# andres-fr/realtime-pose-estimation

Hardware: AMD Instinct MI355X
Metric: images/sec at 640x640 (HRNet-w48 fwd+decode) (higher is better)
Workload: dtype f16 (fp32 accumulate, fp32 BatchNorm; fp32 NCHW in/out); 1 GPU; configs[2]: batch=32 per GPU, 640x640, half-wrapper teacher forward + decode of 17 keypoint channels, weights W0 (seeded random); batch_per_gpu=32, people_per_batch_rank0=960

## Files before the change

realtime-pose-estimation_amd/csrc/conv_mfma.hip:

```cpp
#include <vector>

#include "rtpe_common.h"

namespace rtpe {

typedef _Float16 half8 __attribute__((ext_vector_type(8)));
typedef _Float16 half4 __attribute__((ext_vector_type(4)));
typedef float float4v __attribute__((ext_vector_type(4)));

constexpr int kTapTableBytes = 2048;

__device__ __forceinline__ float round16(float v) { return (float)(_Float16)v; }

template <typename T> struct Prec;
template <> struct Prec<_Float16> {
  static constexpr int EPS = 8;
  static __device__ __forceinline__ float rnd(float v) { return (float)(_Float16)v; }
};
template <> struct Prec<float> {
  static constexpr int EPS = 4;
  static __device__ __forceinline__ float rnd(float v) { return v; }
};

template <typename T>
// ... 532 lines not shown
#define RTPE_CONV_MIXED_VARIANTS(V)                                                                     \
  V(3, 8, 4) V(3, 4, 4) V(3, 2, 4) V(3, 5, 4) V(3, 5, 5) V(4, 4, 4) V(4, 2, 4) V(4, 5, 4) V(4, 5, 5) V(6, 2, 4)   \
  V(2, 8, 4) V(2, 4, 4) V(2, 2, 4) V(2, 5, 4) V(2, 5, 5) V(1, 8, 4) V(1, 4, 4) V(1, 2, 4) V(1, 5, 4) V(1, 5, 5)

static bool conv_has_variant(int mt, int nt, int waves) {
#define RTPE_V(MTv, NTv, Wv) if (mt == MTv && nt == NTv && waves == Wv) return true;
  RTPE_CONV_VARIANTS(RTPE_V)
#undef RTPE_V
  return false;
}

struct TileCand { int waves, nt, th, tw; };
static const TileCand kCands[] = {
    {4, 8, 16, 32}, {4, 8, 32, 16}, {4, 4, 16, 16}, {4, 4, 8, 32}, {4, 4, 32, 8},
    {4, 2, 8, 16},  {4, 2, 16, 8},  {5, 5, 20, 20}, {5, 5, 10, 40}, {5, 5, 40, 10},
    {4, 5, 16, 20}, {4, 5, 20, 16}, {4, 5, 8, 40},  {4, 5, 40, 8},
    {4, 1, 8, 8},
    {2, 2, 8, 8}, {1, 4, 8, 8},
};

static size_t tile_lds(const ConvPlan& p, int th, int tw, int waves, int nt, int mrun = 0) {
  const int hh = (th - 1) * p.in_mul + (p.tapw - 1) * p.dil + 1;
  const size_t in_tile = (size_t)hh * conv_row_pitch(p, tw, 0);
  const size_t out_tile = (size_t)waves * nt * 16 * ((mrun ? (mrun > 0 ? mrun : -mrun) : p.mt) * 16 * p.esize + 16);
  return (size_t)kTapTableBytes + (in_tile > out_tile ? in_tile : out_tile);
}

static bool stream_tile(const ConvPlan& p, const TileCand& c, int N, int H_pos, int W_pos, ConvTile* out,
                        bool allow_resident = true) {
  if (!conv_stream_supports(p) || c.waves < 4) return false;
  if (p.in_mul == 1 ? (c.nt != 4 && c.nt != 5) : (c.nt != (p.mt == 6 ? 1 : 2) || p.n_cchunks != 1)) return false;
  if (p.mt == 6 && p.in_mul != 2) return false;
  const int hh = (c.th - 1) * p.in_mul + 3, hw = (c.tw - 1) * p.in_mul + 3;
  if (hw * 6 > 256) return false;
  const size_t in_tile = (size_t)hh * conv_row_pitch(p, c.tw, 2);
  const size_t out_tile = (size_t)c.waves * c.nt * 16 * (p.mt * 32 + 16);
  size_t buf = in_tile > out_tile ? in_tile : out_tile;
  buf = (buf + 255) / 256 * 256;
  int nw = 3, nb = 3;
  if (allow_resident && p.n_cchunks <= 2 && conv_stream_lds(p, (int)buf, 2, 2 * p.n_cchunks) <= 160 * 1024)
    nw = 2 * p.n_cchunks;
  if (conv_stream_lds(p, (int)buf, nb, nw) > 160 * 1024) nb = 2;
  if (conv_stream_lds(p, (int)buf, nb, nw) > 160 * 1024) return false;
  const long tiles = (long)((H_pos + c.th - 1) / c.th) * ((W_pos + c.tw - 1) / c.tw) * N;
  const long units = tiles * p.n_cb;
  static const int g_env = env_int("RTPE_PERSIST_G", 32);
  long G = g_env;
  const long need = (units + 7) / 8;
  if (G > need) G = need;
  G = (G + p.n_cb - 1) / p.n_cb * p.n_cb;
  memset(out, 0, sizeof(*out));
  out->nt = c.nt; out->waves = c.waves; out->th = c.th; out->tw = c.tw;
  out->kind = 2; out->grid = (int)(8 * G); out->buf_bytes = (int)buf; out->n_bufs = nb;
  out->n_wslots = nw;
  out->lds_bytes = conv_stream_lds(p, (int)buf, nb, nw);
  return true;
}

static ConvTile make_stream_tile(const ConvPlan& p, int N, int H_pos, int W_pos) {
  static const int force_nt = RTPE_DIAG_ENV_INT("RTPE_CONV_NT", 0);
  static const int force_waves = RTPE_DIAG_ENV_INT("RTPE_CONV_WAVES", 0);
  static const int force_th = RTPE_DIAG_ENV_INT("RTPE_CONV_TH", 0);
  double best_score = 1e30;
  ConvTile best;
  memset(&best, 0, sizeof(best));
  for (const TileCand& c : kCands) {
    ConvTile t;
    if ((force_nt && c.nt != force_nt) || (force_waves && c.waves != force_waves) || (force_th && c.th != force_th)) continue;
    if (!stream_tile(p, c, N, H_pos, W_pos, &t)) continue;
    const double waste = (double)((H_pos + c.th - 1) / c.th * c.th) * ((W_pos + c.tw - 1) / c.tw * c.tw) /
                         ((double)H_pos * W_pos);
// ... 39 lines not shown
  static const int stream = getenv("RTPE_CONV_STREAM") ? atoi(getenv("RTPE_CONV_STREAM")) : 1;
  if (allow_stream && (stream & 1) && conv_stream_supports(p)) {
    ConvTile t = make_stream_tile(p, N, H_pos, W_pos);
    if (t.nt) return t;
  }
  static const long lds_cap = getenv("RTPE_CONV_LDS_CAP") ? atol(getenv("RTPE_CONV_LDS_CAP")) : 80 * 1024;
  static const int force_nt = RTPE_DIAG_ENV_INT("RTPE_CONV_NT", 0);
  static const int force_waves = RTPE_DIAG_ENV_INT("RTPE_CONV_WAVES", 0);
  double best_score = 1e30;
  ConvTile best;
  memset(&best, 0, sizeof(best));
  for (const TileCand& c : kCands) {
    if (p.mt == 4 && c.nt == 8) continue;
    if (p.mt == 6 && c.nt > 2) continue;
    if (c.nt == 1 || c.waves < 4) continue;
    if (force_nt && c.nt != force_nt) continue;
    if (force_waves && c.waves != force_waves) continue;
    const size_t lds = tile_lds(p, c.th, c.tw, c.waves, c.nt);
    if (lds > 160 * 1024 || ((long)lds > lds_cap && !(c.nt == 2))) continue;
    const long tiles = (long)((H_pos + c.th - 1) / c.th) * ((W_pos + c.tw - 1) / c.tw);
    const double waste = (double)tiles * c.th * c.tw / ((double)H_pos * W_pos);
    const long wgs = tiles * N * p.n_cb;
    double score = waste;
    if (wgs < 512) score *= 1.0 + 0.25 * (512.0 - wgs) / 512.0;
    score *= 1.0 + 0.4 / c.nt;
    const double halo = (double)((c.th - 1) * p.in_mul + (p.tapw - 1) * p.dil + 1) *
                        ((c.tw - 1) * p.in_mul + (p.tapw - 1) * p.dil + 1) / ((double)c.th * c.tw * p.in_mul * p.in_mul);
    score *= 1.0 + 0.1 * (halo - 1.0);
    if (score < best_score) {
      best_score = score;
// ... 128 lines not shown
      ConvTile st;
      if (stream_tile(p, c, N, H_pos, W_pos, &st)) out->push_back(st);
      if (p.n_cchunks == 2 && st.nt && st.n_wslots != 3 && stream_tile(p, c, N, H_pos, W_pos, &st, false) &&
          st.n_bufs == 3)
        out->push_back(st);
    }
  }
  {
    ConvTile dt;
    if (direct_tile(p, &dt)) out->push_back(dt);
    if (conv64_tile(p, N, H_pos, W_pos, &dt)) out->push_back(dt);
  }
}

int conv_launch(const ConvPlan& p, const ConvTile& t, const ConvArgs& a, hipStream_t s) {
  RTPE_REQUIRE(t.th * t.tw * (t.kind == 0 && t.mrun < 0 ? 2 : 1) == 16 * t.nt * t.waves,
               "conv tile %dx%d != 16*%d*%d", t.th, t.tw, t.nt, t.waves);
  RTPE_REQUIRE(t.lds_bytes <= 160 * 1024, "conv tile needs %zu B of LDS", t.lds_bytes);
  RTPE_REQUIRE(t.kind != 0 || t.lds_bytes >= tile_lds(p, t.th, t.tw, t.waves, t.nt, t.mrun),
               "conv tile (%zu B of LDS) was made for another plan (needs %zu B)", t.lds_bytes,
               tile_lds(p, t.th, t.tw, t.waves, t.nt, t.mrun));
  RTPE_REQUIRE(a.kc * 4 * sizeof(int) <= (size_t)kTapTableBytes, "k chunk table overflow (kc=%d)", a.kc);
  const int eps = 16 / p.esize;
  RTPE_REQUIRE(a.in_ld % eps == 0 && (a.y == nullptr || (a.out_ld % eps == 0 && a.cout_store % eps == 0 &&
                                                         ((uintptr_t)a.y & 15) == 0)),
               "conv: NHWC views must be 16-byte aligned with channel counts that are multiples of %d "
               "(in_ld=%d out_ld=%d cout_store=%d y=%p)", eps, a.in_ld, a.out_ld, a.cout_store, (void*)a.y);
  RTPE_REQUIRE(a.res == nullptr || (a.res_ld % eps == 0 && ((uintptr_t)a.res & 15) == 0), "conv: residual view alignment");
  RTPE_REQUIRE(((uintptr_t)a.x & 15) == 0, "conv: input view must be 16-byte aligned");
  if (t.kind == 2) return conv_stream_launch(p, t, a, s);
  if (t.kind == 4) return conv_direct_launch(p, a, s);
// ... 31 lines not shown
```

realtime-pose-estimation_amd/csrc/conv_stream.hip:

```cpp
#include "conv_stream_dev.h"

namespace rtpe {


constexpr int kResReg0 = 224;
#define RTPE_RES_LOAD(K, R0, R1, R2, R3)                                                             \
  if (it == K)                                                                                       \
    asm volatile("global_load_dwordx4 v[" #R0 ":" #R3 "], %0, %1" ::"v"(off), "s"(rb)               \
                 : "memory", "v" #R0, "v" #R1, "v" #R2, "v" #R3);
#define RTPE_RES_ADD(K, R0, R1, R2, R3)                                                              \
  if (it == K)                                                                                       \
    asm volatile("v_pk_add_f16 %0, %0, v" #R0 "\n\tv_pk_add_f16 %1, %1, v" #R1 "\n\tv_pk_add_f16 %2, %2, v" #R2 \
                 "\n\tv_pk_add_f16 %3, %3, v" #R3                                                   \
                 : "+v"(w[0]), "+v"(w[1]), "+v"(w[2]), "+v"(w[3]));
#define RTPE_RES_ALL(X)                                                                              \
  X(0, 224, 225, 226, 227) X(1, 228, 229, 230, 231) X(2, 232, 233, 234, 235) X(3, 236, 237, 238, 239) \
  X(4, 240, 241, 242, 243) X(5, 244, 245, 246, 247) X(6, 248, 249, 250, 251) X(7, 252, 253, 254, 255)

template <int MT, int NT, int WAVES>
__global__ void __launch_bounds__((WAVES + kLoaders) * 64) __attribute__((amdgpu_num_vgpr(kResReg0)))
conv_stream_kernel(const ConvArgs a) {
  extern __shared__ __attribute__((aligned(16))) char smem[];
  constexpr int WSLOT = MT * kKH * 1024;
  char* const wring = smem;
  const int NWS = a.n_wslots;
  char* const tiles = smem + NWS * WSLOT;
  const int tid = threadIdx.x;
  const int lane = tid & 63;
  const int wv = __builtin_amdgcn_readfirstlane(tid >> 6);

  Units um;
  um.init(a.N * a.tiles_x * a.tiles_y, a.n_cb);
  const uint32_t tiles_xy = (uint32_t)(a.tiles_x * a.tiles_y);
  const int ncc = a.n_cchunks;
  const int sh = __builtin_ctz((unsigned)ncc);
  const int S = um.count << sh;
// ... 150 lines not shown
#endif
    return;
  }

  const int r = lane & 15;
  const int g = lane >> 4;
  int toff[kKC];
#pragma unroll
  for (int k = 0; k < kKC; ++k) {
    int kk = k * 32 + g * 8;
    if (kk >= 9 * kCC) kk -= 9 * kCC;
    const int tap = kk / kCC, c = kk - tap * kCC;
    const int ty = tap / 3, tx = tap - ty * 3;
    toff[k] = ty * a.rowb + tx * kPStride + c * 2;
  }
  int pixbase[NT];
#pragma unroll
  for (int nt = 0; nt < NT; ++nt) {
    const uint32_t p = (wv * NT + nt) * 16 + r;
    const uint32_t oy = fdiv(p, a.div_tw);
    const uint32_t ox = p - oy * a.tw;
    pixbase[nt] = (int)(oy * a.in_mul * a.rowb + ox * a.in_mul * kPStride);
  }
  constexpr int ROWB = MT * 32 + 16;
  constexpr int CH = MT * 2;
  constexpr int NIT = (NT * 16 * CH + 63) / 64;
  int eoff[NIT], epos[NIT];
#pragma unroll
  for (int it = 0; it < NIT; ++it) {
    const int c = it * 64 + lane;
    const int pw = c / CH, slot = c - pw * CH;
    const uint32_t p = wv * NT * 16 + pw;
    const uint32_t oyt = fdiv(p, a.div_tw);
    const uint32_t oxt = p - oyt * a.tw;
    eoff[it] = c < NT * 16 * CH ? pw * ROWB + slot * 16 : 0;
    epos[it] = (int)((oyt << 16) | ((oxt * a.o_mul) << 8) | (slot * 16));
  }
  const uint32_t row_pix = (uint32_t)(a.W_full * a.o_mul) & 0xffffffu;
  auto piece_off = [&](int e, uint32_t ld2) __attribute__((always_inline)) {
    const uint32_t pix = __umul24((uint32_t)e >> 16, row_pix) + (((uint32_t)e >> 8) & 255u);
    return __umul24(pix, ld2) + ((uint32_t)e & 255u);
  };

  float4v acc[MT][NT];
  int bsel = 0;
  int wsel = 0;
  const int n_units = um.count;

  float4v al[MT], be[MT];
  int cb0;
  {
    int tile0;
    um.get(0, &tile0, &cb0);
#pragma unroll
    for (int m = 0; m < MT; ++m) {
      const int c4 = (cb0 * MT + m) * 16 + g * 4;
      al[m] = *reinterpret_cast<const float4v*>(a.alpha + c4);
      be[m] = *reinterpret_cast<const float4v*>(a.beta + c4);
    }
  }
#pragma unroll
  for (int m = 0; m < MT; ++m)
    asm volatile("" ::"v"(al[m]), "v"(be[m]));
  const int cblk = cb0 * MT * 16;
#pragma unroll
  for (int it = 0; it < NIT; ++it) {
    const int c = it * 64 + lane;
    const int slot = c % CH;
    if (c >= NT * 16 * CH || cblk + slot * 8 >= a.cout_store) epos[it] |= 0x7fff0000;
  }
  const bool use_res = a.res != nullptr && !(a.ablate & 2);
#ifdef RTPE_CONV_STAMPS
  unsigned long long st[16] = {0};
  const unsigned long long k_begin = __builtin_readcyclecounter();
#endif

  auto half_stage = [&](const char* wslot, const char* tilebuf, auto hsel) {
    constexpr int H = decltype(hsel)::value;
    const char* wl = wslot + lane * 16;
    half8 af[2][MT], bf[2][NT];
#pragma unroll
    for (int m = 0; m < MT; ++m) af[0][m] = *reinterpret_cast<const half8*>(wl + m * 1024);
#pragma unroll
    for (int nt = 0; nt < NT; ++nt) bf[0][nt] = *reinterpret_cast<const half8*>(tilebuf + pixbase[nt] + toff[H * kKH]);
#pragma unroll
    for (int kk = 0; kk < kKH; ++kk) {
      const int cur = kk & 1, nxt = cur ^ 1;
      if (kk + 1 < kKH) {
#pragma unroll
        for (int m = 0; m < MT; ++m)
          af[nxt][m] = *reinterpret_cast<const half8*>(wl + ((kk + 1) * MT + m) * 1024);
#pragma unroll
        for (int nt = 0; nt < NT; ++nt)
          bf[nxt][nt] = *reinterpret_cast<const half8*>(tilebuf + pixbase[nt] + toff[H * kKH + kk + 1]);
      }
#pragma unroll
      for (int m = 0; m < MT; ++m)
#pragma unroll
        for (int nt = 0; nt < NT; ++nt)
          acc[m][nt] = __builtin_amdgcn_mfma_f32_16x16x32_f16(af[cur][m], bf[cur][nt], acc[m][nt], 0, 0, 0);
      if (kk + 1 < kKH) {
#pragma unroll
        for (int i = 0; i < (MT + NT + 3) / 4; ++i) {
          __builtin_amdgcn_sched_group_barrier(0x008, 1, 0);
          __builtin_amdgcn_sched_group_barrier(0x002, 4, 0);
          __builtin_amdgcn_sched_group_barrier(0x100, 4, 0);
        }
      }
      __builtin_amdgcn_sched_barrier(0);
    }
  };

  struct UnitPos { uint32_t n; int py0, px0; };
  auto unit_pos = [&](int u) {
    int tile, cb;
    um.get(u, &tile, &cb);
    uint32_t t = (uint32_t)tile;
    UnitPos q;
    q.n = fdiv(t, a.div_tiles_xy);
    t -= q.n * tiles_xy;
    const uint32_t tyi = fdiv(t, a.div_tiles_x);
    const uint32_t txi = t - tyi * a.tiles_x;
    q.py0 = (int)tyi * a.th;
    q.px0 = (int)txi * a.tw;
    return q;
  };
  static_assert(NIT <= 8, "residual register window");
  auto load_res = [&](int u) {
    const UnitPos q = unit_pos(u);
    const int hy = a.H_pos - q.py0, hx = (a.W_pos - q.px0) * a.o_mul;
    const size_t pix0 = ((size_t)q.n * a.H_full + q.py0 * a.o_mul + a.oy_add) * a.W_full + q.px0 * a.o_mul + a.ox_add;
    const _Float16* rb = a.res + pix0 * a.res_ld + (size_t)cb0 * a.res_cs;
    const uint32_t ld2 = (uint32_t)a.res_ld * 2u;
#pragma unroll
    for (int it = 0; it < NIT; ++it) {
      int e = epos[it];
      asm volatile("" : "+v"(e));
      const bool ok = (e >> 16) < hy && ((e >> 8) & 255) < hx;
      const uint32_t off = ok ? piece_off(e, ld2) : 0u;
      RTPE_RES_ALL(RTPE_RES_LOAD)
    }
  };

  auto run_unit = [&](int u) {
#ifdef RTPE_CONV_STAMPS
    unsigned long long m0, m1, m2, m3, m4;
#endif
    const UnitPos q = unit_pos(u);
#pragma unroll
    for (int m = 0; m < MT; ++m)
#pragma unroll
      for (int nt = 0; nt < NT; ++nt) acc[m][nt] = float4v{0.f, 0.f, 0.f, 0.f};
    char* tilebuf = nullptr;
    for (int cci = 0; cci < ncc; ++cci) {
      tilebuf = tiles + bsel * a.buf_bytes;
      const int w0 = resident ? 2 * cci : wsel;
      const int w1 = resident ? 2 * cci + 1 : (wsel == 2 ? 0 : wsel + 1);
      SSTAMP(m0);
      RTPE_SBARRIER();
      SSTAMP(m1);
      if (!(a.ablate & 1)) half_stage(wring + w0 * WSLOT, tilebuf, std::integral_constant<int, 0>());
      SSTAMP(m2);
      if (!resident) RTPE_SBARRIER();
      SSTAMP(m3);
      if (!(a.ablate & 1)) half_stage(wring + w1 * WSLOT, tilebuf, std::integral_constant<int, 1>());
      SSTAMP(m4);
#ifdef RTPE_CONV_STAMPS
      st[0] += m1 - m0; st[1] += m2 - m1; st[2] += m3 - m2; st[3] += m4 - m3; st[5] += 1;
#endif
      if (cci + 1 < ncc) {
        bsel = bsel + 1 == NB ? 0 : bsel + 1;
        wsel = wsel == 0 ? 2 : wsel - 1;
      }
    }
    int lane_e = lane;
    asm volatile("" : "+v"(lane_e));
    const int re = lane_e & 15, ge = lane_e >> 4;
    asm volatile("s_waitcnt lgkmcnt(0)" ::: "memory");
    SSTAMP(m0);
    RTPE_SBARRIER();
    SSTAMP(m1);
    char* obuf = tilebuf + wv * (NT * 16 * ROWB);
    auto bn_to_lds = [&](auto rc, auto nchw) {
      constexpr bool RC = decltype(rc)::value, NCHW = decltype(nchw)::value;
#pragma unroll
      for (int nt = 0; nt < NT; ++nt) {
#pragma unroll
        for (int m = 0; m < MT; ++m) {
          const float4v v = acc[m][nt];
          half4 o;
          if (RC) {
            o = bn_round(v, al[m], be[m]);
          } else {
            float2v lo{v[0], v[1]}, hi{v[2], v[3]};
            lo = __builtin_elementwise_fma(lo, float2v{al[m][0], al[m][1]}, float2v{be[m][0], be[m][1]});
            hi = __builtin_elementwise_fma(hi, float2v{al[m][2], al[m][3]}, float2v{be[m][2], be[m][3]});
            const half2v olo = __builtin_convertvector(lo, half2v), ohi = __builtin_convertvector(hi, half2v);
            o = half4{olo[0], olo[1], ohi[0], ohi[1]};
          }
          *reinterpret_cast<half4*>(obuf + (nt * 16 + re) * ROWB + m * 32 + ge * 8) = o;
          if (NCHW) {
            const uint32_t p = (wv * NT + nt) * 16 + re;
            const uint32_t oyt = fdiv(p, a.div_tw);
            const uint32_t oxt = p - oyt * a.tw;
            const int py = q.py0 + (int)oyt, px = q.px0 + (int)oxt;
            if (py < a.H_pos && px < a.W_pos) {
              const int oy = py * a.o_mul + a.oy_add, ox = px * a.o_mul + a.ox_add;
              const int c4 = (cb0 * MT + m) * 16 + ge * 4;
#pragma unroll
              for (int jx = 0; jx < 4; ++jx) {
                const int c = c4 + jx;
                if (c < a.nchw_channels) {
                  const float xr = (float)o[jx];
                  const float x = a.relu ? (xr > 0.f ? xr : 0.f) : xr;
                  const size_t oi = (((size_t)q.n * a.nchw_channels + c) * a.H_full + oy) * a.W_full + ox;
                  if (a.nchw_f32)
                    reinterpret_cast<float*>(a.y_nchw)[oi] = x;
                  else
                    reinterpret_cast<_Float16*>(a.y_nchw)[oi] = (_Float16)x;
                }
              }
            }
          }
        }
      }
    };
    if (a.y_nchw != nullptr) {
      if (a.round_conv) bn_to_lds(std::true_type(), std::true_type()); else bn_to_lds(std::false_type(), std::true_type());
    } else {
      if (a.round_conv) bn_to_lds(std::true_type(), std::false_type()); else bn_to_lds(std::false_type(), std::false_type());
    }
    SSTAMP(m2);
    if (a.y != nullptr && !(a.ablate & 2)) {
      if (use_res) asm volatile("s_waitcnt vmcnt(0)" ::: "memory");
      SSTAMP(m3);
      half8 ov[NIT];
#pragma unroll
      for (int it = 0; it < NIT; ++it) ov[it] = *reinterpret_cast<const half8*>(obuf + eoff[it]);
      const int hy = a.H_pos - q.py0, hx = (a.W_pos - q.px0) * a.o_mul;
      const size_t pix0 = ((size_t)q.n * a.H_full + q.py0 * a.o_mul + a.oy_add) * a.W_full + q.px0 * a.o_mul + a.ox_add;
      char* const yb = reinterpret_cast<char*>(a.y + pix0 * a.out_ld + (size_t)cb0 * a.out_cs);
      const uint32_t ld2 = (uint32_t)a.out_ld * 2u;
#pragma unroll
      for (int it = 0; it < NIT; ++it) {
        if (use_res) {
          int4v w = __builtin_bit_cast(int4v, ov[it]);
          RTPE_RES_ALL(RTPE_RES_ADD)
          ov[it] = __builtin_bit_cast(half8, w);
        }
        if (a.relu) {
          short8 b = __builtin_bit_cast(short8, ov[it]);
          b = b & ~(b >> 15);
          ov[it] = __builtin_bit_cast(half8, b);
        }
      }
      if (use_res && u + 1 < n_units) load_res(u + 1);
#pragma unroll
      for (int it = 0; it < NIT; ++it) {
        int e = epos[it];
        asm volatile("" : "+v"(e));
        if ((e >> 16) < hy && ((e >> 8) & 255) < hx) store16_wt(yb + piece_off(e, ld2), ov[it]);
      }
    }
    asm volatile("s_waitcnt lgkmcnt(0)" ::: "memory");
    SSTAMP(m4);
#ifdef RTPE_CONV_STAMPS
    { unsigned long long m5; SSTAMP(m5);
      st[12] += m1 - m0; st[13] += m2 - m1; st[4] += m3 - m2; st[14] += m4 - m3; st[10] += m5 - m4; }
#endif
    bsel = bsel + 1 == NB ? 0 : bsel + 1;
    wsel = wsel == 0 ? 2 : wsel - 1;
  };

  if ((a.ablate >> 8) && ((blockIdx.x >> 3) & 1))
    for (int i = 0; i < (a.ablate >> 8); ++i) __builtin_amdgcn_s_sleep(16);
  if (use_res) load_res(0);
  for (int u = 0; u < n_units; ++u) run_unit(u);
#ifdef RTPE_CONV_STAMPS
  if (a.dbg != nullptr && lane == 0) {
    st[15] = __builtin_readcyclecounter() - k_begin;
    const int slots[] = {0, 1, 2, 3, 4, 5, 10, 12, 13, 14, 15};
    for (int i : slots) atomicAdd(&a.dbg[i], st[i]);
  }
#endif
}

template <int MT, int NT, int WAVES>
static int launch_stream(const ConvTile& t, const ConvArgs& a, hipStream_t s) {
  static unsigned long long attr_mask = 0;
  auto kern = conv_stream_kernel<MT, NT, WAVES>;
  if (first_use_on_device(&attr_mask)) {
    RTPE_HIP_CHECK(hipFuncSetAttribute(reinterpret_cast<const void*>(kern),
                                       hipFuncAttributeMaxDynamicSharedMemorySize, 160 * 1024));
  }
  hipLaunchKernelGGL(kern, dim3((unsigned)t.grid), dim3((WAVES + kLoaders) * 64), t.lds_bytes, s, a);
  RTPE_HIP_CHECK(hipGetLastError());
  return RTPE_OK;
}

size_t conv_stream_lds(const ConvPlan& p, int buf_bytes, int n_bufs, int n_wslots) {
  return (size_t)n_wslots * p.mt * kKH * 1024 + (size_t)n_bufs * buf_bytes;
}

bool conv_stream_supports(const ConvPlan& p) {
  return p.esize == 2 && p.dil == 1 && p.cc == kCC && p.pstride == kPStride && p.tapw == 3 && p.kc == kKC &&
         (p.in_mul == 1 || p.in_mul == 2) && (p.mt <= 3 || (p.mt == 6 && p.in_mul == 2 && p.n_cchunks == 1)) &&
         (p.n_cchunks & (p.n_cchunks - 1)) == 0;
}

int conv_stream_launch(const ConvPlan& p, const ConvTile& t, const ConvArgs& a, hipStream_t s) {
  RTPE_REQUIRE(conv_stream_supports(p), "streaming conv: unsupported plan");
  RTPE_REQUIRE(a.x_bytes > 0 && a.x_bytes < 0x80000000ull, "streaming conv: input view of %zu bytes", (size_t)a.x_bytes);
  RTPE_REQUIRE(a.cin % 8 == 0 && (a.in_ld >= a.cin ? a.in_cs == kCC : a.in_ld == kCC && a.in_cs >= kCC),
               "streaming conv: cin=%d in_ld=%d chunk stride %lld", a.cin, a.in_ld, a.in_cs);
  RTPE_REQUIRE(t.grid >= 8 && t.grid % 8 == 0 && (t.grid / 8) % p.n_cb == 0, "streaming conv: bad grid %d", t.grid);
  RTPE_REQUIRE((t.n_bufs == 2 || t.n_bufs == 3) && t.buf_bytes % 16 == 0 &&
               (t.n_wslots == 3 || t.n_wslots == 2 * p.n_cchunks) &&
               t.lds_bytes >= conv_stream_lds(p, t.buf_bytes, t.n_bufs, t.n_wslots) && t.lds_bytes <= 160 * 1024,
               "streaming conv: LDS layout (%d buffers of %d B, %d weight slots, %zu B)", t.n_bufs, t.buf_bytes,
               t.n_wslots, t.lds_bytes);
  RTPE_REQUIRE(a.halo_w * kSlots <= 256, "streaming conv: halo row of %d pixels", a.halo_w);
  RTPE_REQUIRE(a.rowb >= a.halo_w * kPStride && (size_t)a.halo_h * a.rowb <= (size_t)t.buf_bytes &&
               (size_t)t.waves * t.nt * 16 * (p.mt * 32 + 16) <= (size_t)t.buf_bytes, "streaming conv: tile buffer too small");
#define RTPE_S(MTv, NTv, Wv) \
  if (p.mt == MTv && t.nt == NTv && t.waves == Wv) return launch_stream<MTv, NTv, Wv>(t, a, s);
  RTPE_S(3, 4, 4) RTPE_S(3, 5, 4) RTPE_S(3, 5, 5) RTPE_S(3, 2, 4) RTPE_S(6, 1, 4)
  RTPE_S(2, 4, 4) RTPE_S(2, 5, 4) RTPE_S(2, 5, 5)
  RTPE_S(1, 4, 4) RTPE_S(1, 5, 4) RTPE_S(1, 5, 5)
#undef RTPE_S
  set_error("streaming conv: no kernel variant mt=%d nt=%d waves=%d", p.mt, t.nt, t.waves);
  return RTPE_E_INVALID;
}

}
```

realtime-pose-estimation_amd/csrc/engine.hip:

```cpp
#include <stdarg.h>

#include <chrono>
#include <mutex>
#include <map>
#include <tuple>
#include <vector>

#include "rtpe_common.h"

namespace rtpe {

static thread_local std::string g_err;

void set_error(const char* fmt, ...) {
  char buf[1024];
  va_list ap;
  va_start(ap, fmt);
  vsnprintf(buf, sizeof(buf), fmt, ap);
  va_end(ap);
  g_err = buf;
}

int hip_fail(hipError_t e, const char* what, const char* file, int line) {
  set_error("HIP error %d (%s) at %s:%d: %s", (int)e, hipGetErrorString(e), file, line, what);
// ... 54 lines not shown
  size_t arena_bytes;
  int n_preds, n_refined;
  std::mutex lane_mu;
  hipStream_t lane_stream[4] = {nullptr, nullptr, nullptr, nullptr};
  std::vector<hipEvent_t> op_event;
  std::vector<char> needs_event;
  std::vector<std::vector<int>> wait_ops;
  hipEvent_t fork_event = nullptr;
  bool has_regions = false;
  bool any_size = false;
};

static size_t align_up(size_t v, size_t a) { return (v + a - 1) / a * a; }

namespace rtpe {
static int g_options[kNumOptions] = {-1, -1, -1, -1, -1, -1, -1, -1, -1, -1, -1, -1};
static const char* const kOptionNames[kNumOptions] = {"block_ring", "block_pc", "direct_1x1", "lanes", "tile_dma", "pair_1x1", "fused_stem", "conv64", "head_direct", "deconv48", "conv48s2", "pair_proj"};
static const char* const kOptionEnv[kNumOptions] = {"RTPE_BLOCK_RING", "RTPE_BLOCK_PC", "RTPE_DIRECT_1X1", "RTPE_LANES", "RTPE_TILE_DMA", "RTPE_PAIR_1X1", "RTPE_FUSED_STEM", "RTPE_CONV64", "RTPE_HEAD_DIRECT", "RTPE_DECONV48", "RTPE_CONV48S2", "RTPE_PAIR_PROJ"};
static const int kOptionDefault[kNumOptions] = {0, 1, 1, 1, 1, 1, 1, 1, 1, 1, 1, 1};
int get_option(int key) {
  int v = __atomic_load_n(&g_options[key], __ATOMIC_RELAXED);
  if (v < 0) {
    v = kOptionEnv[key][0] ? env_int(kOptionEnv[key], kOptionDefault[key]) : kOptionDefault[key];
    __atomic_store_n(&g_options[key], v, __ATOMIC_RELAXED);
  }
  return v;
}
}

extern "C" int rtpe_set_option(const char* name, int32_t value) {
  RTPE_REQUIRE(name != nullptr && value >= 0, "set_option: bad argument");
  for (int k = 0; k < kNumOptions; ++k)
    if (kOptionNames[k][0] && strcmp(name, kOptionNames[k]) == 0) {
      __atomic_store_n(&g_options[k], (int)value, __ATOMIC_RELAXED);
// ... 400 lines not shown
    if (!(plane[d.in_t] || plane[d.out_t] || (d.res_t >= 0 && plane[d.res_t]))) continue;
    const rtpe_tensor_desc& ti = h->tensors[d.in_t];
    const ConvTile t = (tuned && (*tuned)[i * 4].nt) ? (*tuned)[i * 4]
                                                      : conv_make_tile(o.plan[0], N, extent(H, ti.ds_log2), extent(W, ti.ds_log2));
    if (t.kind != 2) {
      plane[d.in_t] = plane[d.out_t] = 0;
      if (d.res_t >= 0) plane[d.res_t] = 0;
    }
  }
  return plane;
}

struct RouteOpts {
  int fused_stem = get_option(kOptFusedStem), pair_1x1 = get_option(kOptPair1x1), pair_proj = get_option(kOptPairProj),
      conv64 = get_option(kOptConv64), head_direct = get_option(kOptHeadDirect), deconv48 = get_option(kOptDeconv48),
      conv48s2 = get_option(kOptConv48s2);
};

struct Fwd {
  const rtpe_hrnet* h;
  int N, H, W;
  char* base;
  void *preds, *refined;
  int out_dtype;
  std::vector<size_t> offs;
  size_t ws_need;
  const std::vector<ConvTile>* tuned = nullptr;
  std::vector<char> plane;
  bool rag;
  const int32_t* ext;
  const int32_t* level(int ds) const { return ext + (size_t)ds * 2 * N; }
// ... 86 lines not shown
static ConvArgs conv_op_args(const Fwd& f, size_t i, int k, const ConvTile& t) {
  ConvArgs a = conv_op_args(f, i, k);
  conv_fill_args(f.h->ops[i].geom[k], f.h->ops[i].plan[k], t, &a);
  return a;
}

static bool conv_direct_ok(const ConvArgs& a) {
  return a.x_bytes < 0x80000000ull && a.y != nullptr && a.y_nchw == nullptr && a.o_mul == 1;
}

static void conv_fix_tile(const RouteOpts& opt, const ConvPlan& p, const ConvArgs& a, bool plane_io, ConvTile* t) {
  const bool direct_ok = conv_direct_ok(a);
  if (t->kind == 4 && !direct_ok) *t = conv_make_tile(p, a.N, a.H_pos, a.W_pos, false);
  if (t->kind == 5 && !(direct_ok && a.res == nullptr && !plane_io && opt.conv64 != 0))
    *t = conv_make_tile(p, a.N, a.H_pos, a.W_pos, true, false);
}

static int conv_pick(const RouteOpts& opt, const ConvPlan& p, const ConvTile& t, const ConvArgs& a, bool plane_io) {
  if (opt.head_direct != 0 && conv_head_supports(p, a)) return kRouteHead;
  if (opt.conv48s2 != 0 && !plane_io && conv48s2_supports(p, a)) return kRouteS2;
  return t.kind == 2 ? kRouteStream : t.kind == 4 ? kRouteDirect : t.kind == 5 ? kRouteConv64 : kRouteTile;
}

static bool deconv_merges(const ConvPlan* p, const ConvTile& tile0) {
  static const int merge_deconv = env_int("RTPE_DECONV_MERGE", 1);
  bool merge = merge_deconv && tile0.kind == 0;
  for (int k = 1; k < 4 && merge; ++k)
    merge = p[k].mt == p[0].mt && p[k].cc == p[0].cc && p[k].kc == p[0].kc && p[k].n_cchunks == p[0].n_cchunks &&
            p[k].n_cb == p[0].n_cb && p[k].pstride == p[0].pstride && p[k].tapw == p[0].tapw;
  return merge;
// ... 1099 lines not shown
```

realtime-pose-estimation_amd/csrc/rtpe_common.h:

```cpp
#pragma once
#include <hip/hip_runtime.h>
#include <hip/hip_fp16.h>
#include <stdint.h>
#include <stdio.h>
#include <stdlib.h>
#include <string.h>
#include <string>
#include <vector>

#include "rtpe_hip.h"

namespace rtpe {

void set_error(const char* fmt, ...);
int hip_fail(hipError_t e, const char* what, const char* file, int line);

#define RTPE_HIP_CHECK(expr)                                               \
  do {                                                                     \
    hipError_t _e = (expr);                                                \
    if (_e != hipSuccess) return ::rtpe::hip_fail(_e, #expr, __FILE__, __LINE__); \
  } while (0)

#define RTPE_REQUIRE(cond, ...)                 \
  do {                                          \
// ... 1 lines not shown
      ::rtpe::set_error(__VA_ARGS__);           \
      return RTPE_E_INVALID;                    \
    }                                           \
  } while (0)

inline int env_int(const char* name, int dflt) {
  const char* v = getenv(name);
  return v ? atoi(v) : dflt;
}
#ifdef RTPE_DIAG
#define RTPE_DIAG_ENV_INT(name, dflt) ::rtpe::env_int(name, dflt)
#else
#define RTPE_DIAG_ENV_INT(name, dflt) (dflt)
#endif

enum { kOptBlockRing = 0, kOptBlockPC = 1, kOptDirect1x1 = 2, kOptLanes = 3, kOptTileDma = 4, kOptPair1x1 = 5, kOptFusedStem = 6, kOptConv64 = 7, kOptHeadDirect = 8, kOptDeconv48 = 9, kOptConv48s2 = 10, kOptPairProj = 11, kNumOptions = 12 };
int get_option(int key);

inline bool first_use_on_device(unsigned long long* mask) {
  int dev = 0;
  if (hipGetDevice(&dev) != hipSuccess || dev < 0 || dev > 63) return true;
  const unsigned long long bit = 1ull << dev;
  const unsigned long long old = __atomic_fetch_or(mask, bit, __ATOMIC_RELAXED);
  return !(old & bit);
}

struct DeviceGuard {
  int prev = -1;
  bool switched = false;
  hipError_t err = hipSuccess;
  explicit DeviceGuard(int device) {
// ... 130 lines not shown
  int deconv_class;
  int esize;
  int dil;
};

ConvPlan conv_make_plan(const ConvGeom& g);
ConvTile conv_make_tile(const ConvPlan& p, int N, int H_pos, int W_pos, bool allow_direct = true, bool allow_conv64 = true,
                        bool allow_stream = true);
int conv_row_pitch(const ConvPlan& p, int tw, int kind);
bool conv_deint(const ConvPlan& p, int kind);
void conv_enum_tiles(const ConvPlan& p, int N, int H_pos, int W_pos, std::vector<ConvTile>* out);
void conv_pack_weights(const ConvGeom& g, const ConvPlan& p, const void* w, void* packed);
void conv_fill_args(const ConvGeom& g, const ConvPlan& p, const ConvTile& t, ConvArgs* a);
int conv_launch(const ConvPlan& p, const ConvTile& t, const ConvArgs& a, hipStream_t s);
bool conv_stream_supports(const ConvPlan& p);
size_t conv_stream_lds(const ConvPlan& p, int buf_bytes, int n_bufs, int n_wslots);
int conv_stream_launch(const ConvPlan& p, const ConvTile& t, const ConvArgs& a, hipStream_t s);
bool conv_pair_supports(int cin1, int cout1, int cout2);
int conv_pair_launch(const ConvPlan& p1, const ConvArgs& c1, const ConvPlan& p2, const ConvArgs& c2, hipStream_t s,
                     const ConvPlan* pd = nullptr, const ConvArgs* cd = nullptr);
int conv_direct_mb(const ConvPlan& p);
bool conv64_supports(const ConvPlan& p);
size_t conv64_lds();
int conv64_grid(int N, int H_pos, int W_pos);
int conv64_launch(const ConvPlan& p, const ConvTile& t, const ConvArgs& a, hipStream_t s);
int conv_direct_launch(const ConvPlan& p, const ConvArgs& a, hipStream_t s);
bool conv_head_supports(const ConvPlan& p, const ConvArgs& a);
int conv_head_launch(const ConvPlan& p, const ConvArgs& a, hipStream_t s);
bool deconv48_supports(const ConvPlan& p, const ConvArgs& merged);
int deconv48_launch(const ConvPlan& p, const ConvArgs& merged, hipStream_t s);
// ... 80 lines not shown
```

Measured before the change: 2395 images/sec.

## Add split streaming-conv tile using four waves for 400-pixel 48-channel tiles

Adds a split variant of the streaming 3x3 conv kernel for stride-1, 48-channel cout blocks. Four compute waves each take six 16-pixel column tiles, and the leftover 25th column tile is spread across three waves, one cout subtile each, using a rotated weight order. This replaces the five-wave 20x20-style tiles with four waves and drops a wave per workgroup. The cost is an extra MFMA stream per wave, a late residual and BN load, and extra LDS for the odd slab. The option is on by default and swaps in via a resplit when a five-wave tile was chosen.

```diff
diff --git a/realtime-pose-estimation_amd/csrc/conv_mfma.hip b/realtime-pose-estimation_amd/csrc/conv_mfma.hip
--- a/realtime-pose-estimation_amd/csrc/conv_mfma.hip
+++ b/realtime-pose-estimation_amd/csrc/conv_mfma.hip
@@ -570,6 +570,7 @@
 static const TileCand kCands[] = {
     {4, 8, 16, 32}, {4, 8, 32, 16}, {4, 4, 16, 16}, {4, 4, 8, 32}, {4, 4, 32, 8},
     {4, 2, 8, 16},  {4, 2, 16, 8},  {5, 5, 20, 20}, {5, 5, 10, 40}, {5, 5, 40, 10},
+    {4, kStreamSplitNt, 20, 20}, {4, kStreamSplitNt, 10, 40}, {4, kStreamSplitNt, 40, 10},
     {4, 5, 16, 20}, {4, 5, 20, 16}, {4, 5, 8, 40},  {4, 5, 40, 8},
     {4, 1, 8, 8},
     {2, 2, 8, 8}, {1, 4, 8, 8},
@@ -583,14 +584,18 @@
 }
 
 static bool stream_tile(const ConvPlan& p, const TileCand& c, int N, int H_pos, int W_pos, ConvTile* out,
-                        bool allow_resident = true) {
+                        bool allow_resident = true, int split_mode = -1) {
   if (!conv_stream_supports(p) || c.waves < 4) return false;
-  if (p.in_mul == 1 ? (c.nt != 4 && c.nt != 5) : (c.nt != (p.mt == 6 ? 1 : 2) || p.n_cchunks != 1)) return false;
+  const bool split = c.nt == kStreamSplitNt;
+  if (split && !(p.in_mul == 1 && p.mt == 3)) return false;
+  if (p.in_mul == 1 && p.mt == 3 && (split || c.waves == 5) &&
+      split != ((split_mode < 0 ? get_option(kOptStreamSplit) : split_mode) != 0)) return false;
+  if (p.in_mul == 1 ? (c.nt != 4 && c.nt != 5 && !split) : (c.nt != (p.mt == 6 ? 1 : 2) || p.n_cchunks != 1)) return false;
   if (p.mt == 6 && p.in_mul != 2) return false;
   const int hh = (c.th - 1) * p.in_mul + 3, hw = (c.tw - 1) * p.in_mul + 3;
   if (hw * 6 > 256) return false;
   const size_t in_tile = (size_t)hh * conv_row_pitch(p, c.tw, 2);
-  const size_t out_tile = (size_t)c.waves * c.nt * 16 * (p.mt * 32 + 16);
+  const size_t out_tile = conv_stream_slab(p, c.waves, c.nt);
   size_t buf = in_tile > out_tile ? in_tile : out_tile;
   buf = (buf + 255) / 256 * 256;
   int nw = 3, nb = 3;
@@ -611,6 +616,20 @@
   out->n_wslots = nw;
   out->lds_bytes = conv_stream_lds(p, (int)buf, nb, nw);
   return true;
+}
+
+void conv_stream_resplit(const ConvPlan& p, int N, int H_pos, int W_pos, bool split, ConvTile* t) {
+  if (t->kind != 2 || p.in_mul != 1 || p.mt != 3) return;
+  const bool is = conv_stream_is_split(*t);
+  if (is == split || (!is && t->waves != 5)) return;
+  for (const TileCand& c : kCands) {
+    if (c.th != t->th || c.tw != t->tw || (c.nt == kStreamSplitNt) != split || (!split && c.waves != 5)) continue;
+    ConvTile n;
+    if (stream_tile(p, c, N, H_pos, W_pos, &n, t->n_wslots != 3, split ? 1 : 0)) {
+      *t = n;
+      return;
+    }
+  }
 }
 
 static ConvTile make_stream_tile(const ConvPlan& p, int N, int H_pos, int W_pos) {
@@ -680,6 +699,7 @@
     if (p.mt == 4 && c.nt == 8) continue;
     if (p.mt == 6 && c.nt > 2) continue;
     if (c.nt == 1 || c.waves < 4) continue;
+    if (c.nt == kStreamSplitNt) continue;
     if (force_nt && c.nt != force_nt) continue;
     if (force_waves && c.waves != force_waves) continue;
     const size_t lds = tile_lds(p, c.th, c.tw, c.waves, c.nt);
@@ -838,7 +858,7 @@
 }
 
 int conv_launch(const ConvPlan& p, const ConvTile& t, const ConvArgs& a, hipStream_t s) {
-  RTPE_REQUIRE(t.th * t.tw * (t.kind == 0 && t.mrun < 0 ? 2 : 1) == 16 * t.nt * t.waves,
+  RTPE_REQUIRE(t.th * t.tw * (t.kind == 0 && t.mrun < 0 ? 2 : 1) == 16 * (t.nt * t.waves + (conv_stream_is_split(t) ? 1 : 0)),
                "conv tile %dx%d != 16*%d*%d", t.th, t.tw, t.nt, t.waves);
   RTPE_REQUIRE(t.lds_bytes <= 160 * 1024, "conv tile needs %zu B of LDS", t.lds_bytes);
   RTPE_REQUIRE(t.kind != 0 || t.lds_bytes >= tile_lds(p, t.th, t.tw, t.waves, t.nt, t.mrun),
diff --git a/realtime-pose-estimation_amd/csrc/conv_stream.hip b/realtime-pose-estimation_amd/csrc/conv_stream.hip
--- a/realtime-pose-estimation_amd/csrc/conv_stream.hip
+++ b/realtime-pose-estimation_amd/csrc/conv_stream.hip
@@ -17,9 +17,11 @@
   X(0, 224, 225, 226, 227) X(1, 228, 229, 230, 231) X(2, 232, 233, 234, 235) X(3, 236, 237, 238, 239) \
   X(4, 240, 241, 242, 243) X(5, 244, 245, 246, 247) X(6, 248, 249, 250, 251) X(7, 252, 253, 254, 255)
 
-template <int MT, int NT, int WAVES>
+constexpr int kSplitRowB = 48;
+template <int MT, int NT, int WAVES, bool SPLIT = false>
 __global__ void __launch_bounds__((WAVES + kLoaders) * 64) __attribute__((amdgpu_num_vgpr(kResReg0)))
 conv_stream_kernel(const ConvArgs a) {
+  static_assert(!SPLIT || MT == 3, "the odd column tile is split by cout tile over three waves");
   extern __shared__ __attribute__((aligned(16))) char smem[];
   constexpr int WSLOT = MT * kKH * 1024;
   char* const wring = smem;
@@ -200,10 +202,15 @@
     const int ty = tap / 3, tx = tap - ty * 3;
     toff[k] = ty * a.rowb + tx * kPStride + c * 2;
   }
-  int pixbase[NT];
-#pragma unroll
-  for (int nt = 0; nt < NT; ++nt) {
-    const uint32_t p = (wv * NT + nt) * 16 + r;
+  constexpr int NBF = NT + (SPLIT ? 1 : 0);
+  const int mx = wv < MT - 1 ? wv : MT - 1;
+  auto rot = [&](int m) __attribute__((always_inline)) {
+    return !SPLIT ? m : mx + m >= MT ? mx + m - MT : mx + m;
+  };
+  int pixbase[NBF];
+#pragma unroll
+  for (int nt = 0; nt < NBF; ++nt) {
+    const uint32_t p = (SPLIT && nt == NT ? WAVES * NT : wv * NT + nt) * 16 + r;
     const uint32_t oy = fdiv(p, a.div_tw);
     const uint32_t ox = p - oy * a.tw;
     pixbase[nt] = (int)(oy * a.in_mul * a.rowb + ox * a.in_mul * kPStride);
@@ -228,7 +235,16 @@
     return __umul24(pix, ld2) + ((uint32_t)e & 255u);
   };
 
+  int wrot[MT];
+  if constexpr (SPLIT) {
+#pragma unroll
+    for (int m = 0; m < MT; ++m) {
+      wrot[m] = lane * 16 + rot(m) * 1024;
+      asm volatile("" : "+v"(wrot[m]));
+    }
+  }
   float4v acc[MT][NT];
+  float4v accx;
   int bsel = 0;
   int wsel = 0;
   const int n_units = um.count;
@@ -238,16 +254,21 @@
   {
     int tile0;
     um.get(0, &tile0, &cb0);
+  }
+  auto load_bn = [&]() __attribute__((always_inline)) {
 #pragma unroll
     for (int m = 0; m < MT; ++m) {
-      const int c4 = (cb0 * MT + m) * 16 + g * 4;
+      const int c4 = (cb0 * MT + (SPLIT ? rot(m) : m)) * 16 + g * 4;
       al[m] = *reinterpret_cast<const float4v*>(a.alpha + c4);
       be[m] = *reinterpret_cast<const float4v*>(a.beta + c4);
     }
-  }
-#pragma unroll
-  for (int m = 0; m < MT; ++m)
-    asm volatile("" ::"v"(al[m]), "v"(be[m]));
+  };
+  if constexpr (!SPLIT) {
+    load_bn();
+#pragma unroll
+    for (int m = 0; m < MT; ++m)
+      asm volatile("" ::"v"(al[m]), "v"(be[m]));
+  }
   const int cblk = cb0 * MT * 16;
 #pragma unroll
   for (int it = 0; it < NIT; ++it) {
@@ -255,6 +276,14 @@
     const int slot = c % CH;
     if (c >= NT * 16 * CH || cblk + slot * 8 >= a.cout_store) epos[it] |= 0x7fff0000;
   }
+  int xpos = 0x7fff0000;
+  if (SPLIT) {
+    const int slot = mx * 2 + (lane & 1);
+    const uint32_t p = WAVES * NT * 16 + (lane >> 1);
+    const uint32_t oyt = fdiv(p, a.div_tw);
+    const uint32_t oxt = p - oyt * a.tw;
+    if (lane < 32 && wv < MT && cblk + slot * 8 < a.cout_store) xpos = (int)((oyt << 16) | ((oxt * a.o_mul) << 8) | (slot * 16));
+  }
   const bool use_res = a.res != nullptr && !(a.ablate & 2);
 #ifdef RTPE_CONV_STAMPS
   unsigned long long st[16] = {0};
@@ -264,20 +293,30 @@
   auto half_stage = [&](const char* wslot, const char* tilebuf, auto hsel) {
     constexpr int H = decltype(hsel)::value;
     const char* wl = wslot + lane * 16;
-    half8 af[2][MT], bf[2][NT];
-#pragma unroll
-    for (int m = 0; m < MT; ++m) af[0][m] = *reinterpret_cast<const half8*>(wl + m * 1024);
-#pragma unroll
-    for (int nt = 0; nt < NT; ++nt) bf[0][nt] = *reinterpret_cast<const half8*>(tilebuf + pixbase[nt] + toff[H * kKH]);
+    const char* wlr[MT];
+    if constexpr (SPLIT) {
+#pragma unroll
+      for (int m = 0; m < MT; ++m) wlr[m] = wslot + wrot[m];
+    }
+    half8 af[2][MT], bf[2][NBF];
+#pragma unroll
+    for (int m = 0; m < MT; ++m) {
+      if constexpr (SPLIT) af[0][m] = *reinterpret_cast<const half8*>(wlr[m]);
+      else af[0][m] = *reinterpret_cast<const half8*>(wl + m * 1024);
+    }
+#pragma unroll
+    for (int nt = 0; nt < NBF; ++nt) bf[0][nt] = *reinterpret_cast<const half8*>(tilebuf + pixbase[nt] + toff[H * kKH]);
 #pragma unroll
     for (int kk = 0; kk < kKH; ++kk) {
       const int cur = kk & 1, nxt = cur ^ 1;
       if (kk + 1 < kKH) {
 #pragma unroll
-        for (int m = 0; m < MT; ++m)
-          af[nxt][m] = *reinterpret_cast<const half8*>(wl + ((kk + 1) * MT + m) * 1024);
-#pragma unroll
-        for (int nt = 0; nt < NT; ++nt)
+        for (int m = 0; m < MT; ++m) {
+          if constexpr (SPLIT) af[nxt][m] = *reinterpret_cast<const half8*>(wlr[m] + (kk + 1) * MT * 1024);
+          else af[nxt][m] = *reinterpret_cast<const half8*>(wl + ((kk + 1) * MT + m) * 1024);
+        }
+#pragma unroll
+        for (int nt = 0; nt < NBF; ++nt)
           bf[nxt][nt] = *reinterpret_cast<const half8*>(tilebuf + pixbase[nt] + toff[H * kKH + kk + 1]);
       }
 #pragma unroll
@@ -285,9 +324,10 @@
 #pragma unroll
         for (int nt = 0; nt < NT; ++nt)
           acc[m][nt] = __builtin_amdgcn_mfma_f32_16x16x32_f16(af[cur][m], bf[cur][nt], acc[m][nt], 0, 0, 0);
+      if constexpr (SPLIT) accx = __builtin_amdgcn_mfma_f32_16x16x32_f16(af[cur][0], bf[cur][NT], accx, 0, 0, 0);
       if (kk + 1 < kKH) {
 #pragma unroll
-        for (int i = 0; i < (MT + NT + 3) / 4; ++i) {
+        for (int i = 0; i < (MT + NBF + 3) / 4; ++i) {
           __builtin_amdgcn_sched_group_barrier(0x008, 1, 0);
           __builtin_amdgcn_sched_group_barrier(0x002, 4, 0);
           __builtin_amdgcn_sched_group_barrier(0x100, 4, 0);
@@ -311,7 +351,12 @@
     q.px0 = (int)txi * a.tw;
     return q;
   };
-  static_assert(NIT <= 8, "residual register window");
+  static_assert(SPLIT ? NIT == 9 : NIT <= 8, "residual register window");
+  constexpr int NWIN = NIT < 8 ? NIT : 8;
+  auto res_base = [&](const UnitPos& q) {
+    const size_t pix0 = ((size_t)q.n * a.H_full + q.py0 * a.o_mul + a.oy_add) * a.W_full + q.px0 * a.o_mul + a.ox_add;
+    return a.res + pix0 * a.res_ld + (size_t)cb0 * a.res_cs;
+  };
   auto load_res = [&](int u) {
     const UnitPos q = unit_pos(u);
     const int hy = a.H_pos - q.py0, hx = (a.W_pos - q.px0) * a.o_mul;
@@ -319,7 +364,7 @@
     const _Float16* rb = a.res + pix0 * a.res_ld + (size_t)cb0 * a.res_cs;
     const uint32_t ld2 = (uint32_t)a.res_ld * 2u;
 #pragma unroll
-    for (int it = 0; it < NIT; ++it) {
+    for (int it = 0; it < NWIN; ++it) {
       int e = epos[it];
       asm volatile("" : "+v"(e));
       const bool ok = (e >> 16) < hy && ((e >> 8) & 255) < hx;
@@ -337,6 +382,7 @@
     for (int m = 0; m < MT; ++m)
 #pragma unroll
       for (int nt = 0; nt < NT; ++nt) acc[m][nt] = float4v{0.f, 0.f, 0.f, 0.f};
+    accx = float4v{0.f, 0.f, 0.f, 0.f};
     char* tilebuf = nullptr;
     for (int cci = 0; cci < ncc; ++cci) {
       tilebuf = tiles + bsel * a.buf_bytes;
@@ -359,6 +405,21 @@
         wsel = wsel == 0 ? 2 : wsel - 1;
       }
     }
+    int4v late[2] = {int4v{0, 0, 0, 0}, int4v{0, 0, 0, 0}};
+    if constexpr (SPLIT) {
+      load_bn();
+      if (use_res) {
+        const int ry = a.H_pos - q.py0, rx = (a.W_pos - q.px0) * a.o_mul;
+        const char* rb = reinterpret_cast<const char*>(res_base(q));
+        const uint32_t ld2 = (uint32_t)a.res_ld * 2u;
+        int e8 = epos[NIT - 1], ex = xpos;
+        asm volatile("" : "+v"(e8), "+v"(ex));
+        const uint32_t o8 = ((e8 >> 16) < ry && ((e8 >> 8) & 255) < rx) ? piece_off(e8, ld2) : 0u;
+        const uint32_t ox = ((ex >> 16) < ry && ((ex >> 8) & 255) < rx) ? piece_off(ex, ld2) : 0u;
+        late[0] = *reinterpret_cast<const int4v*>(rb + o8);
+        late[1] = *reinterpret_cast<const int4v*>(rb + ox);
+      }
+    }
     int lane_e = lane;
     asm volatile("" : "+v"(lane_e));
     const int re = lane_e & 15, ge = lane_e >> 4;
@@ -367,8 +428,23 @@
     RTPE_SBARRIER();
     SSTAMP(m1);
     char* obuf = tilebuf + wv * (NT * 16 * ROWB);
+    char* xbuf = tilebuf + WAVES * (NT * 16 * ROWB) + wv * (16 * kSplitRowB);
     auto bn_to_lds = [&](auto rc, auto nchw) {
       constexpr bool RC = decltype(rc)::value, NCHW = decltype(nchw)::value;
+      if constexpr (SPLIT) {
+        const float4v alx = al[0], bex = be[0];
+        half4 o;
+        if (RC) {
+          o = bn_round(accx, alx, bex);
+        } else {
+          float2v lo{accx[0], accx[1]}, hi{accx[2], accx[3]};
+          lo = __builtin_elementwise_fma(lo, float2v{alx[0], alx[1]}, float2v{bex[0], bex[1]});
+          hi = __builtin_elementwise_fma(hi, float2v{alx[2], alx[3]}, float2v{bex[2], bex[3]});
+          const half2v olo = __builtin_convertvector(lo, half2v), ohi = __builtin_convertvector(hi, half2v);
+          o = half4{olo[0], olo[1], ohi[0], ohi[1]};
+        }
+        *reinterpret_cast<half4*>(xbuf + re * kSplitRowB + ge * 8) = o;
+      }
 #pragma unroll
       for (int nt = 0; nt < NT; ++nt) {
 #pragma unroll
@@ -384,7 +460,7 @@
             const half2v olo = __builtin_convertvector(lo, half2v), ohi = __builtin_convertvector(hi, half2v);
             o = half4{olo[0], olo[1], ohi[0], ohi[1]};
           }
-          *reinterpret_cast<half4*>(obuf + (nt * 16 + re) * ROWB + m * 32 + ge * 8) = o;
+          *reinterpret_cast<half4*>(obuf + (nt * 16 + re) * ROWB + (SPLIT ? rot(m) : m) * 32 + ge * 8) = o;
           if (NCHW) {
             const uint32_t p = (wv * NT + nt) * 16 + re;
             const uint32_t oyt = fdiv(p, a.div_tw);
@@ -392,7 +468,7 @@
             const int py = q.py0 + (int)oyt, px = q.px0 + (int)oxt;
             if (py < a.H_pos && px < a.W_pos) {
               const int oy = py * a.o_mul + a.oy_add, ox = px * a.o_mul + a.ox_add;
-              const int c4 = (cb0 * MT + m) * 16 + ge * 4;
+              const int c4 = (cb0 * MT + (SPLIT ? rot(m) : m)) * 16 + ge * 4;
 #pragma unroll
               for (int jx = 0; jx < 4; ++jx) {
                 const int c = c4 + jx;
@@ -422,7 +498,17 @@
       SSTAMP(m3);
       half8 ov[NIT];
 #pragma unroll
-      for (int it = 0; it < NIT; ++it) ov[it] = *reinterpret_cast<const half8*>(obuf + eoff[it]);
+      for (int it = 0; it < NIT; ++it) {
+        if constexpr (SPLIT) {
+          const int c = it * 64 + lane_e;
+          const int pw = c / CH;
+          ov[it] = *reinterpret_cast<const half8*>(obuf + pw * ROWB + (c - pw * CH) * 16);
+        } else {
+          ov[it] = *reinterpret_cast<const half8*>(obuf + eoff[it]);
+        }
+      }
+      half8 ovx;
+      if constexpr (SPLIT) ovx = *reinterpret_cast<const half8*>(xbuf + ((lane_e & 31) >> 1) * kSplitRowB + (lane_e & 1) * 16);
       const int hy = a.H_pos - q.py0, hx = (a.W_pos - q.px0) * a.o_mul;
       const size_t pix0 = ((size_t)q.n * a.H_full + q.py0 * a.o_mul + a.oy_add) * a.W_full + q.px0 * a.o_mul + a.ox_add;
       char* const yb = reinterpret_cast<char*>(a.y + pix0 * a.out_ld + (size_t)cb0 * a.out_cs);
@@ -433,6 +519,7 @@
           int4v w = __builtin_bit_cast(int4v, ov[it]);
           RTPE_RES_ALL(RTPE_RES_ADD)
           ov[it] = __builtin_bit_cast(half8, w);
+          if (SPLIT && it >= NWIN) ov[it] = ov[it] + __builtin_bit_cast(half8, late[it - NWIN]);
         }
         if (a.relu) {
           short8 b = __builtin_bit_cast(short8, ov[it]);
@@ -440,6 +527,14 @@
           ov[it] = __builtin_bit_cast(half8, b);
         }
       }
+      if constexpr (SPLIT) {
+        if (use_res) ovx = ovx + __builtin_bit_cast(half8, late[1]);
+        if (a.relu) {
+          short8 b = __builtin_bit_cast(short8, ovx);
+          b = b & ~(b >> 15);
+          ovx = __builtin_bit_cast(half8, b);
+        }
+      }
       if (use_res && u + 1 < n_units) load_res(u + 1);
 #pragma unroll
       for (int it = 0; it < NIT; ++it) {
@@ -447,6 +542,11 @@
         asm volatile("" : "+v"(e));
         if ((e >> 16) < hy && ((e >> 8) & 255) < hx) store16_wt(yb + piece_off(e, ld2), ov[it]);
       }
+      if constexpr (SPLIT) {
+        int e = xpos;
+        asm volatile("" : "+v"(e));
+        if ((e >> 16) < hy && ((e >> 8) & 255) < hx) store16_wt(yb + piece_off(e, ld2), ovx);
+      }
     }
     asm volatile("s_waitcnt lgkmcnt(0)" ::: "memory");
     SSTAMP(m4);
@@ -471,10 +571,10 @@
 #endif
 }
 
-template <int MT, int NT, int WAVES>
+template <int MT, int NT, int WAVES, bool SPLIT = false>
 static int launch_stream(const ConvTile& t, const ConvArgs& a, hipStream_t s) {
   static unsigned long long attr_mask = 0;
-  auto kern = conv_stream_kernel<MT, NT, WAVES>;
+  auto kern = conv_stream_kernel<MT, NT, WAVES, SPLIT>;
   if (first_use_on_device(&attr_mask)) {
     RTPE_HIP_CHECK(hipFuncSetAttribute(reinterpret_cast<const void*>(kern),
                                        hipFuncAttributeMaxDynamicSharedMemorySize, 160 * 1024));
@@ -482,6 +582,10 @@
   hipLaunchKernelGGL(kern, dim3((unsigned)t.grid), dim3((WAVES + kLoaders) * 64), t.lds_bytes, s, a);
   RTPE_HIP_CHECK(hipGetLastError());
   return RTPE_OK;
+}
+
+size_t conv_stream_slab(const ConvPlan& p, int waves, int nt) {
+  return (size_t)waves * nt * 16 * (p.mt * 32 + 16) + (nt == kStreamSplitNt ? (size_t)waves * 16 * kSplitRowB : 0);
 }
 
 size_t conv_stream_lds(const ConvPlan& p, int buf_bytes, int n_bufs, int n_wslots) {
@@ -507,7 +611,12 @@
                t.n_wslots, t.lds_bytes);
   RTPE_REQUIRE(a.halo_w * kSlots <= 256, "streaming conv: halo row of %d pixels", a.halo_w);
   RTPE_REQUIRE(a.rowb >= a.halo_w * kPStride && (size_t)a.halo_h * a.rowb <= (size_t)t.buf_bytes &&
-               (size_t)t.waves * t.nt * 16 * (p.mt * 32 + 16) <= (size_t)t.buf_bytes, "streaming conv: tile buffer too small");
+               conv_stream_slab(p, t.waves, t.nt) <= (size_t)t.buf_bytes, "streaming conv: tile buffer too small");
+  if (conv_stream_is_split(t)) {
+    RTPE_REQUIRE(p.mt == 3 && p.in_mul == 1 && t.waves == 4 && t.th * t.tw == 16 * (t.waves * t.nt + 1) && a.y_nchw == nullptr,
+                 "streaming conv: the split shape takes stride-1 layers of 48-channel cout blocks with an NHWC output");
+    return launch_stream<3, 6, 4, true>(t, a, s);
+  }
 #define RTPE_S(MTv, NTv, Wv) \
   if (p.mt == MTv && t.nt == NTv && t.waves == Wv) return launch_stream<MTv, NTv, Wv>(t, a, s);
   RTPE_S(3, 4, 4) RTPE_S(3, 5, 4) RTPE_S(3, 5, 5) RTPE_S(3, 2, 4) RTPE_S(6, 1, 4)
diff --git a/realtime-pose-estimation_amd/csrc/engine.hip b/realtime-pose-estimation_amd/csrc/engine.hip
--- a/realtime-pose-estimation_amd/csrc/engine.hip
+++ b/realtime-pose-estimation_amd/csrc/engine.hip
@@ -92,10 +92,10 @@
 static size_t align_up(size_t v, size_t a) { return (v + a - 1) / a * a; }
 
 namespace rtpe {
-static int g_options[kNumOptions] = {-1, -1, -1, -1, -1, -1, -1, -1, -1, -1, -1, -1};
-static const char* const kOptionNames[kNumOptions] = {"block_ring", "block_pc", "direct_1x1", "lanes", "tile_dma", "pair_1x1", "fused_stem", "conv64", "head_direct", "deconv48", "conv48s2", "pair_proj"};
-static const char* const kOptionEnv[kNumOptions] = {"RTPE_BLOCK_RING", "RTPE_BLOCK_PC", "RTPE_DIRECT_1X1", "RTPE_LANES", "RTPE_TILE_DMA", "RTPE_PAIR_1X1", "RTPE_FUSED_STEM", "RTPE_CONV64", "RTPE_HEAD_DIRECT", "RTPE_DECONV48", "RTPE_CONV48S2", "RTPE_PAIR_PROJ"};
-static const int kOptionDefault[kNumOptions] = {0, 1, 1, 1, 1, 1, 1, 1, 1, 1, 1, 1};
+static int g_options[kNumOptions] = {-1, -1, -1, -1, -1, -1, -1, -1, -1, -1, -1, -1, -1};
+static const char* const kOptionNames[kNumOptions] = {"block_ring", "block_pc", "direct_1x1", "lanes", "tile_dma", "pair_1x1", "fused_stem", "conv64", "head_direct", "deconv48", "conv48s2", "pair_proj", "stream_split"};
+static const char* const kOptionEnv[kNumOptions] = {"RTPE_BLOCK_RING", "RTPE_BLOCK_PC", "RTPE_DIRECT_1X1", "RTPE_LANES", "RTPE_TILE_DMA", "RTPE_PAIR_1X1", "RTPE_FUSED_STEM", "RTPE_CONV64", "RTPE_HEAD_DIRECT", "RTPE_DECONV48", "RTPE_CONV48S2", "RTPE_PAIR_PROJ", "RTPE_STREAM_SPLIT"};
+static const int kOptionDefault[kNumOptions] = {0, 1, 1, 1, 1, 1, 1, 1, 1, 1, 1, 1, 1};
 int get_option(int key) {
   int v = __atomic_load_n(&g_options[key], __ATOMIC_RELAXED);
   if (v < 0) {
@@ -526,7 +526,7 @@
 struct RouteOpts {
   int fused_stem = get_option(kOptFusedStem), pair_1x1 = get_option(kOptPair1x1), pair_proj = get_option(kOptPairProj),
       conv64 = get_option(kOptConv64), head_direct = get_option(kOptHeadDirect), deconv48 = get_option(kOptDeconv48),
-      conv48s2 = get_option(kOptConv48s2);
+      conv48s2 = get_option(kOptConv48s2), stream_split = get_option(kOptStreamSplit);
 };
 
 struct Fwd {
@@ -643,6 +643,7 @@
   if (t->kind == 4 && !direct_ok) *t = conv_make_tile(p, a.N, a.H_pos, a.W_pos, false);
   if (t->kind == 5 && !(direct_ok && a.res == nullptr && !plane_io && opt.conv64 != 0))
     *t = conv_make_tile(p, a.N, a.H_pos, a.W_pos, true, false);
+  conv_stream_resplit(p, a.N, a.H_pos, a.W_pos, opt.stream_split != 0 && a.y_nchw == nullptr, t);
 }
 
 static int conv_pick(const RouteOpts& opt, const ConvPlan& p, const ConvTile& t, const ConvArgs& a, bool plane_io) {
diff --git a/realtime-pose-estimation_amd/csrc/rtpe_common.h b/realtime-pose-estimation_amd/csrc/rtpe_common.h
--- a/realtime-pose-estimation_amd/csrc/rtpe_common.h
+++ b/realtime-pose-estimation_amd/csrc/rtpe_common.h
@@ -39,7 +39,7 @@
 #define RTPE_DIAG_ENV_INT(name, dflt) (dflt)
 #endif
 
-enum { kOptBlockRing = 0, kOptBlockPC = 1, kOptDirect1x1 = 2, kOptLanes = 3, kOptTileDma = 4, kOptPair1x1 = 5, kOptFusedStem = 6, kOptConv64 = 7, kOptHeadDirect = 8, kOptDeconv48 = 9, kOptConv48s2 = 10, kOptPairProj = 11, kNumOptions = 12 };
+enum { kOptBlockRing = 0, kOptBlockPC = 1, kOptDirect1x1 = 2, kOptLanes = 3, kOptTileDma = 4, kOptPair1x1 = 5, kOptFusedStem = 6, kOptConv64 = 7, kOptHeadDirect = 8, kOptDeconv48 = 9, kOptConv48s2 = 10, kOptPairProj = 11, kOptStreamSplit = 12, kNumOptions = 13 };
 int get_option(int key);
 
 inline bool first_use_on_device(unsigned long long* mask) {
@@ -200,6 +200,10 @@
 void conv_fill_args(const ConvGeom& g, const ConvPlan& p, const ConvTile& t, ConvArgs* a);
 int conv_launch(const ConvPlan& p, const ConvTile& t, const ConvArgs& a, hipStream_t s);
 bool conv_stream_supports(const ConvPlan& p);
+constexpr int kStreamSplitNt = 6;
+inline bool conv_stream_is_split(const ConvTile& t) { return t.kind == 2 && t.nt == kStreamSplitNt; }
+size_t conv_stream_slab(const ConvPlan& p, int waves, int nt);
+void conv_stream_resplit(const ConvPlan& p, int N, int H_pos, int W_pos, bool split, ConvTile* t);
 size_t conv_stream_lds(const ConvPlan& p, int buf_bytes, int n_bufs, int n_wslots);
 int conv_stream_launch(const ConvPlan& p, const ConvTile& t, const ConvArgs& a, hipStream_t s);
 bool conv_pair_supports(int cin1, int cout1, int cout2);
```

Result: slower. 2354 images/sec (-1.7%).
